# indygreg/python-zstandard

Hardware: AMD Instinct MI355X
Metric: GB/s uncompressed throughput, batch decompress of 128 KiB level-3 frames (the decompress half of BASELINE.json's metric; the compress half on the same inputs is this line's 'compress' object) (higher is better)
Workload: dtype u8

## Files before the change

python-zstandard_amd/csrc/zhip_decode_kernel.hpp:

```cpp
#pragma once
#include "zhip_device.hpp"
#include "zhip_format.hpp"
#include "zhip_xxh64.hpp"

#if defined(ZHIP_EMU) && defined(ZD_TRACE)
#include <stdio.h>
extern "C" { extern long zd_trace_pos; extern long zd_cur_frame; extern long zd_stat[16]; }
#define ZD_STAT(i, v) do { if (zh_lane() == 0) zd_stat[i] += (v); } while (0)
#define ZD_TRR(lo, n, what, a1, a2) do { if (zh_lane() == 0 && zd_trace_pos + 40 >= (long)(lo) && zd_trace_pos < (long)(lo) + (long)(n) + 40) fprintf(stderr, "[trace] f%ld range [%ld,+%ld) %s %ld %ld\n", zd_cur_frame, (long)(lo), (long)(n), what, (long)(a1), (long)(a2)); } while (0)
#define ZD_TR(pos, what, a1, a2, a3) do { if ((long)(pos) == zd_trace_pos) fprintf(stderr, "[trace] f%ld pos=%ld %s lane=%u %ld %ld %ld\n", zd_cur_frame, (long)(pos), what, zh_lane(), (long)(a1), (long)(a2), (long)(a3)); } while (0)
#else
#define ZD_TR(pos, what, a1, a2, a3) do { } while (0)
#define ZD_TRR(lo, n, what, a1, a2) do { } while (0)
#define ZD_STAT(i, v) do { } while (0)
#endif
#define ZD_STAGE_BYTES 512
#define ZD_ASM_BYTES 4096
#define ZD_COOP_LEN 32

ZH_CONST uint32_t zc_llBase[36] = {0,1,2,3,4,5,6,7,8,9,10,11,12,13,14,15,16,18,20,22,24,28,32,40,48,64,128,256,512,
                                   1024,2048,4096,8192,16384,32768,65536};
ZH_CONST uint8_t zc_llBits[36] = {0,0,0,0,0,0,0,0,0,0,0,0,0,0,0,0,1,1,1,1,2,2,3,3,4,6,7,8,9,10,11,12,13,14,15,16};
ZH_CONST uint32_t zc_mlBase[53] = {3,4,5,6,7,8,9,10,11,12,13,14,15,16,17,18,19,20,21,22,23,24,25,26,27,28,29,30,31,32,
                                   33,34,35,37,39,41,43,47,51,59,67,83,99,131,259,515,1027,2051,4099,8195,16387,32771,65539};
// ... 254 lines not shown
}
ZH_DEV bool zd_pb_init(ZdPBits& b, const uint8_t* src, uint32_t size)
{
    b.start = src; b.end = src + size; b.ptr = src; b.c = 0; b.d = 0; b.used = 64;
    if (size == 0) return false;
    const uint32_t last = src[size - 1];
    if (last == 0) return false;
    const uint32_t pad = 8 - (uint32_t)zh_highbit32(last);
    if (size >= 8) { b.ptr = src + size - 8; b.c = zh_ld64(b.ptr); b.used = pad; }
    else {
        uint64_t c = 0;
        for (uint32_t i = 0; i < size; i++) c |= (uint64_t)src[i] << (8 * i);
        b.c = c; b.used = pad + (8 - size) * 8;
    }
    b.d = zd_pb_below(b);
    return true;
}
ZH_DEV void zd_pb_norm(ZdPBits& b)
{
    uint32_t nb = b.used >> 3;
    const uint32_t room = (uint32_t)(b.ptr - b.start);
    if (nb > room) nb = room;
    if (nb > 8) nb = 8;
    if (nb) {
        b.c = nb == 8 ? b.d : ((b.c << (8 * nb)) | (b.d >> (64 - 8 * nb)));
        b.ptr -= nb; b.used -= nb * 8;
        b.d = zd_pb_below(b);
    }
}
ZH_DEV uint32_t zd_pb_peek(const ZdPBits& b, uint32_t n) { return (uint32_t)((b.c << (b.used & 63)) >> (64 - n)); }
ZH_DEV bool zd_pb_done(const ZdPBits& b) { return b.ptr == b.start && b.used == 64; }

ZH_DEV bool zd_weights_dist_ok(uint32_t tl, uint32_t maxS) { return tl <= 6 && maxS <= 12 && !(tl == 6 && maxS == 12); }
ZH_DEVFN int zd_read_huf_weights(ZdLDS& L, const uint8_t* src, uint32_t srcSize, uint32_t* pCount, uint32_t* pLog, const ZpPre* pre = nullptr, uint32_t at = 0)
{
    const uint32_t lane = zh_lane();
    if (srcSize < 1) return -ZE_CORRUPTION;
    uint32_t hb = src[0], n, used;
    if (hb >= 128) {
        n = hb - 127; used = 1 + (n + 1) / 2;
        if (used > srcSize) return -ZE_CORRUPTION;
        for (uint32_t i = lane; i < n; i += 64) {
            uint32_t v = src[1 + i / 2];
            L.weights[i] = (uint8_t)((i & 1) ? (v & 15) : (v >> 4));
        }
    } else {
        used = 1 + hb;
        if (used > srcSize || hb < 2) return -ZE_CORRUPTION;
        if (pre && pre->wCount && pre->wAt == at) {
            n = pre->wCount;
            zh_sync();
            ((uint32_t*)L.weights)[lane] = ((const uint32_t*)pre->weights)[lane];
#ifdef ZHIP_EMU
            if (lane == 0) zd_stat[10]++;
#endif
        } else {
        uint8_t* const stg = (uint8_t*)L.u.huf + 4096;
        zh_sync();
        zd_stage_wave(stg, src + 1, hb);
        zh_sync();
        if (lane == 0) {
            uint32_t maxS = 255 > 63 ? 63 : 255, tl = 0;
            int r = zd_read_ncount(L, stg, stg + hb, &maxS, &tl);
            L.misc[0] = (uint32_t)r; L.misc[1] = maxS; L.misc[2] = tl;
        }
        zh_sync();
// ... 3 lines not shown
        if (lane == 0) {
            ZdBits b; uint32_t cnt = 0; int bad = 0;
            if (!zd_bits_init(b, stg + r, hb - (uint32_t)r)) bad = 1;
            else {
                zd_bits_reload(b);
                uint32_t s1 = zd_bits_peek(b, tl); b.used += tl;
                uint32_t s2 = zd_bits_peek(b, tl); b.used += tl;
                if (tl == 0) { s1 = s2 = 0; }
                int64_t left;
                for (;;) {
                    if (b.used >= 32) zd_bits_reload(b);
                    left = (int64_t)(b.ptr - b.start) * 8 + 64 - (int64_t)b.used;
                    uint32_t e1 = L.u.b.wfse[s1], nb1 = (e1 >> 10) & 15;
                    if (cnt > 253) { bad = 1; break; }
                    L.weights[cnt++] = (uint8_t)(e1 >> 19);
                    uint32_t v1 = nb1 ? zd_bits_peek(b, nb1) : 0; b.used += nb1; left -= nb1;
                    s1 = (e1 & 1023) + v1;
                    uint32_t e2 = L.u.b.wfse[s2], nb2 = (e2 >> 10) & 15;
                    if (left < 0) { L.weights[cnt++] = (uint8_t)(e2 >> 19); break; }
                    if (cnt > 253) { bad = 1; break; }
                    L.weights[cnt++] = (uint8_t)(e2 >> 19);
                    uint32_t v2 = nb2 ? zd_bits_peek(b, nb2) : 0; b.used += nb2; left -= nb2;
                    s2 = (e2 & 1023) + v2;
                    if (left < 0) { L.weights[cnt++] = (uint8_t)(L.u.b.wfse[s1] >> 19); break; }
                }
            }
            L.misc[0] = bad ? 0xFFFFFFFFu : cnt;
        }
        zh_sync();
        n = L.misc[0];
        if (n == 0xFFFFFFFFu || n == 0) return -ZE_CORRUPTION;
        }
    }
    zh_sync();
    uint32_t part = 0, ones = 0;
    for (uint32_t i = lane; i < n; i += 64) {
        uint32_t w = L.weights[i];
        if (w > 12) part = 0x02000000u;
        else if (w) part += 1u << (w - 1);
        ones += (w == 1);
    }
    uint32_t total = zh_shfl(zh_scan_add(part), 63);
    uint32_t nOnes = zh_shfl(zh_scan_add(ones), 63);
    if (total == 0 || total >= 0x02000000u) return -ZE_CORRUPTION;
    uint32_t log = (uint32_t)zh_highbit32(total) + 1;
    if (log > 12) return -ZE_CORRUPTION;
    uint32_t rest = (1u << log) - total;
    if (rest & (rest - 1)) return -ZE_CORRUPTION;
    uint32_t lastW = (uint32_t)zh_highbit32(rest) + 1;
    nOnes += (lastW == 1);
    if (nOnes < 2 || (nOnes & 1)) return -ZE_CORRUPTION;
    if (lane == 0) L.weights[n] = (uint8_t)lastW;
    zh_sync();
    *pCount = n + 1; *pLog = log;
    return (int)used;
}

ZH_DEVFN int zd_build_huf(ZdLDS& L, uint32_t count)
{
    const uint32_t lane = zh_lane();
    const uint64_t lt = zh_lt_mask();
    uint32_t wt[4], myStart[4];
    uint32_t part = 0;
    for (int k = 0; k < 4; k++) {
        uint32_t s = (uint32_t)k * 64 + lane;
        wt[k] = s < count ? L.weights[s] : 0;
        if (wt[k]) part += 1u << (wt[k] - 1);
        myStart[k] = 0;
    }
    uint32_t total = zh_shfl(zh_scan_add(part), 63);
    if (total == 0 || (total & (total - 1))) return -ZE_CORRUPTION;
    uint32_t log = (uint32_t)zh_highbit32(total);
    if (log > 12 || log == 0) return -ZE_CORRUPTION;
    zh_sync();
    uint32_t base = 0;
    for (uint32_t w = 1; w <= 12; w++) {
        uint32_t before = 0;
        for (int k = 0; k < 4; k++) {
            uint64_t m = zh_ballot(wt[k] == w);
            if (wt[k] == w) myStart[k] = base + ((before + (uint32_t)zh_popc64(m & lt)) << (w - 1));
            before += (uint32_t)zh_popc64(m);
        }
        base += before << (w - 1);
    }
    for (int k = 0; k < 4; k++) {
        if (!wt[k]) continue;
        uint32_t len = 1u << (wt[k] - 1);
// ... 144 lines not shown
ZH_DEVFN int zd_seq_table(ZdLDS& L, uint32_t mode, int kind, uint32_t* pLog, const uint8_t* p, const uint8_t* end, const ZpPre* pre = nullptr)
{
    const uint32_t lane = zh_lane();
    uint32_t* table = L.fse + (kind == ZD_KIND_LL ? ZD_FSE_LL : kind == ZD_KIND_ML ? ZD_FSE_ML : ZD_FSE_OF);
    const uint32_t maxSym = kind == ZD_KIND_LL ? ZF_MAXLL : kind == ZD_KIND_ML ? ZF_MAXML : ZF_MAXOFF;
    const uint32_t maxLog = kind == ZD_KIND_LL ? ZF_LL_LOGMAX : kind == ZD_KIND_ML ? ZF_ML_LOGMAX : ZF_OF_LOGMAX;
    if (mode == 0) {
        zh_sync();
        if (kind == ZD_KIND_LL) L.norm[lane] = lane < 36 ? zc_llDef[lane] : (int16_t)0;
        else if (kind == ZD_KIND_ML) L.norm[lane] = lane < 53 ? zc_mlDef[lane] : (int16_t)0;
        else L.norm[lane] = lane < 29 ? zc_ofDef[lane] : (int16_t)0;
        uint32_t lg = kind == ZD_KIND_OF ? 5 : 6;
        uint32_t ms = kind == ZD_KIND_LL ? 35 : kind == ZD_KIND_ML ? 52 : 28;
        if (zd_build_fse(L, table, ms, lg, kind) < 0) return -ZE_CORRUPTION;
        *pLog = lg; return 0;
    }
    if (mode == 1) {
        if (p >= end) return -ZE_SRC_SIZE_WRONG;
        uint32_t s = p[0];
        if (s > maxSym) return -ZE_CORRUPTION;
        zh_sync();
        if (lane == 0) {
            uint32_t extra = kind == ZD_KIND_LL ? L.llBits[s] : kind == ZD_KIND_ML ? L.mlBits[s] : s;
            table[0] = ZD_CELL(0, 0, extra, s);
        }
        zh_sync();
        *pLog = 0; return 1;
    }
    if (mode == 2) {
        zh_sync();
        int r; uint32_t ms, tl;
        if (pre && pre->t[kind].valid) {
            L.norm[lane] = pre->norm[kind][lane];
            r = (int)pre->t[kind].used; ms = pre->t[kind].maxSym; tl = pre->t[kind].log;
#ifdef ZHIP_EMU
            if (lane == 0) zd_stat[11]++;
#endif
        } else {
            if (lane == 0) {
                uint32_t ms0 = maxSym, tl0 = 0;
                int r0 = zd_read_ncount(L, p, end, &ms0, &tl0);
                L.misc[0] = (uint32_t)r0; L.misc[1] = ms0; L.misc[2] = tl0;
            }
            zh_sync();
            r = (int)L.misc[0]; ms = L.misc[1]; tl = L.misc[2];
        }
        if (r < 0 || tl > maxLog) return -ZE_CORRUPTION;
        if (zd_build_fse(L, table, ms, tl, kind) < 0) return -ZE_CORRUPTION;
        *pLog = tl; return r;
    }
    if (*pLog == 0xFF) return -ZE_CORRUPTION;
    return 0;
}

ZH_DEV uint32_t zd_hist_byte(const uint8_t* dst, const uint8_t* dictEnd, int32_t pos)
{
    return pos >= 0 ? dst[pos] : dictEnd[pos];
}

ZH_COLD void zd_match_wave(uint8_t* dst, const uint8_t* dictEnd, uint32_t mdst, uint32_t off, uint32_t ml)
{
    const uint32_t lane = zh_lane();
    const int32_t sbeg = (int32_t)mdst - (int32_t)off;
    if (off >= 64) {
        for (uint32_t c = 0; c < ml; c += 64) {
            uint32_t j = c + lane;
            if (j < ml) dst[mdst + j] = (uint8_t)zd_hist_byte(dst, dictEnd, sbeg + (int32_t)j);
// ... 492 lines not shown
```

python-zstandard_amd/csrc/zhip_decode_pipeline.hpp:

```cpp
#pragma once
#include "zhip_decode_kernel.hpp"

ZH_DEV void zp_pack_fse(ZdLDS& L, uint32_t* T, uint32_t llLog, uint32_t ofLog, uint32_t mlLog)
{
    const uint32_t lane = zh_lane();
    for (uint32_t u = lane; u < ZP_FSE_CELLS / 2; u += 64) {
        const uint32_t lg = u < 256 ? llLog : u < 512 ? mlLog : ofLog;
        const uint32_t local = (2 * u) & (u < 512 ? 511u : 255u);
        uint32_t pair = 0;
        for (uint32_t k = 0; k < 2; k++) {
            uint32_t cell = 0;
            if (local + k < (1u << lg)) {
                const uint32_t e = L.fse[2 * u + k];
                cell = ((e >> 19) << 10) | (((e & 1023) + (1u << lg)) >> ((e >> 10) & 15));
            }
            pair |= cell << (16 * k);
        }
        T[u] = pair;
    }
}

struct ZpHdr { uint32_t pos, blockMax, hasChecksum, skippable; uint64_t fcs; };
ZH_DEV int zp_frame_header(const ZhipPipeArgs& a, const uint8_t* src, uint32_t srcSize, ZpHdr& h)
{
    const uint32_t mg = a.magicless ? 0u : 4u;
    h.skippable = 0;
    if (srcSize < mg + 1) return ZE_SRC_SIZE_WRONG;
    if (mg && (zh_ld32(src) & 0xFFFFFFF0u) == ZF_MAGIC_SKIPPABLE) {
        if (srcSize < 8 || (uint64_t)zh_ld32(src + 4) + 8 > srcSize) return ZE_SRC_SIZE_WRONG;
        h.skippable = 1; h.pos = 0; h.blockMax = 0; h.hasChecksum = 0; h.fcs = 0;
        return 0;
    }
    if (mg && zh_ld32(src) != ZF_MAGIC) return ZE_PREFIX_UNKNOWN;
    const uint32_t fhd = src[mg];
// ... 76 lines not shown
        if (modes & 3) return ZE_CORRUPTION;
        const bool allShared = share && de && (modes >> 2) == 0x3F;
        if (allShared) {
            st.llLog = de->llLog; st.ofLog = de->ofLog; st.mlLog = de->mlLog;
            if (sp >= send) return ZE_CORRUPTION;
        } else {
            if (de && !dictInLds) {
                zh_sync();
                const uint32_t* T = a.dictTables->fse;
                if ((modes >> 6) == 3) { for (uint32_t k = lane; k < (1u << de->llLog); k += 64) L.fse[ZD_FSE_LL + k] = T[ZD_FSE_LL + k]; st.llLog = de->llLog; }
                if (((modes >> 4) & 3) == 3) { for (uint32_t k = lane; k < (1u << de->ofLog); k += 64) L.fse[ZD_FSE_OF + k] = T[ZD_FSE_OF + k]; st.ofLog = de->ofLog; }
                if (((modes >> 2) & 3) == 3) { for (uint32_t k = lane; k < (1u << de->mlLog); k += 64) L.fse[ZD_FSE_ML + k] = T[ZD_FSE_ML + k]; st.mlLog = de->mlLog; }
                zh_sync();
            }
            const uint32_t hn = (uint32_t)(send - sp) < 256u ? (uint32_t)(send - sp) : 256u;
            uint8_t* const stg = (uint8_t*)L.u.huf + 4096;
            zh_sync();
            zd_stage_wave(stg, sp, hn);
            zh_sync();
            const uint8_t* lp = stg; const uint8_t* const lend = stg + hn;
            const ZpPre* const spre = df.pre && df.pre->seqAt == (uint32_t)(sp - (src + pos)) ? df.pre : nullptr;
            int q = zd_seq_table(L, modes >> 6, ZD_KIND_LL, &st.llLog, lp, lend, spre); if (q < 0) return -q; sp += q; lp += q;
            q = zd_seq_table(L, (modes >> 4) & 3, ZD_KIND_OF, &st.ofLog, lp, lend, spre); if (q < 0) return -q; sp += q; lp += q;
            q = zd_seq_table(L, (modes >> 2) & 3, ZD_KIND_ML, &st.mlLog, lp, lend, spre); if (q < 0) return -q; sp += q; lp += q;
            if (sp >= send) return ZE_CORRUPTION;
            zh_sync();
            uint32_t* const T = (uint32_t*)(a.fseTables + (size_t)t * ZP_FSE_CELLS);
            zp_pack_fse(L, T, st.llLog, st.ofLog, st.mlLog);
        }
        m.logs = st.llLog | (st.ofLog << 8) | (st.mlLog << 16) | (allShared ? ZP_LOGS_SHARED : 0u);
    }
    m.seqOff = (uint32_t)(sp - src); m.seqEnd = pos + bs;
    ZD_T(P, ZP_SEQTAB);
    return 0;
}

ZH_DEV void zp_enter_bins(const ZhipPipeArgs& a, ZdMeta& m)
{
    const uint32_t ks = m.nbSeq ? 1u + (m.nbSeq >> ZP_BIN_SHIFT) : 0u;
    const uint32_t kl = (m.litMode & 255u) == 3u ? 1u + (m.litSize >> ZP_LITBIN_SHIFT) : 0u;
    if (ks) m.pad = zh_atomic_add(a.counters + ZP_CNT_BINS + (256 - (ks > 256 ? 256u : ks)), 1u);
    if (kl) m.hasChecksum |= zh_atomic_add(a.counters + ZP_CNT_BINS + 256 + (256 - (kl > 256 ? 256u : kl)), 1u) << 1;
}
ZH_DEV void zp_enter_bins_wave(const ZhipPipeArgs& a, ZdMeta& m, bool on)
{
    const uint32_t lane = zh_lane();
    const uint32_t ks = on && m.nbSeq ? 1u + (m.nbSeq >> ZP_BIN_SHIFT) : 0u;
    const uint32_t kl = on && (m.litMode & 255u) == 3u ? 1u + (m.litSize >> ZP_LITBIN_SHIFT) : 0u;
    const uint32_t bS = ks ? 256u - (ks > 256u ? 256u : ks) : 0xFFFFu, bL = kl ? 256u + (256u - (kl > 256u ? 256u : kl)) : 0xFFFFu;
#pragma unroll
    for (int which = 0; which < 2; which++) {
        const uint32_t mine = which ? bL : bS;
        uint64_t todo = zh_ballot(mine != 0xFFFFu);
        while (todo) {
            const uint32_t leader = (uint32_t)zh_ctz64(todo);
            const uint32_t b = zh_shfl(mine, leader);
            const uint64_t same = zh_ballot(mine == b);
            uint32_t base = 0;
            if (lane == leader) base = zh_atomic_add(a.counters + ZP_CNT_BINS + b, (uint32_t)zh_popc64(same));
            base = zh_shfl(base, leader);
            if (mine == b) { const uint32_t rank = base + (uint32_t)zh_popc64(same & zh_lt_mask()); if (which) m.hasChecksum |= rank << 1; else m.pad = rank; }
            todo &= ~same;
        }
    }
}
ZH_DEV void zp_meta_clear(ZdMeta& m)
// ... 87 lines not shown
        const bool done = mine && zp_lit_shared_try(a, a.first + i, m, need16);
        const uint32_t n16 = done ? need16 : 0u;
        const uint32_t incl = zh_scan_add(n16), total = zh_shfl(incl, 63);
        uint32_t lb = 0;
        if (total) lb = zh_first(zh_atomic_add(a.counters + 8, lane == 0 ? total : 0u)) + incl - n16;
        const bool noRoom = done && n16 && (uint64_t)lb + n16 > a.arenaBudget16;
        zp_enter_bins_wave(a, m, done && !noRoom);
        if (a.ckLater) {
            const uint32_t nck = (uint32_t)zh_popc64(zh_ballot(done && !noRoom && (m.hasChecksum & 1u)));
            anyCk |= nck != 0;
        }
        if (done) {
            if (noRoom) {
                const uint32_t bm = m.blockMax, lo = m.fcsLo, hi = m.fcsHi;
                zp_meta_clear(m); m.blockMax = bm; m.fcsLo = lo; m.fcsHi = hi; m.path = 2;
                a.meta[i] = m;
                const uint32_t k = zh_atomic_add(a.fallbackCount, 1u); a.fallbackList[k] = a.first + i;
            } else {
                a.bases[2 * (size_t)i + 1] = n16 ? a.arenaBudget16 - lb - n16 : 0u;
                a.meta[i] = m;
#ifdef ZHIP_EMU
                zd_stat[7]++;
#endif
            }
        }
        const uint64_t rest = zh_ballot(mine && !done);
        if (rest) {
            const uint32_t at = zh_first(zh_atomic_add(a.counters + 10, lane == 0 ? (uint32_t)zh_popc64(rest) : 0u));
            if (mine && !done) a.order[at + (uint32_t)zh_popc64(rest & zh_lt_mask())] = i;
        }
    }
}

struct ZpPreLane { int16_t wnorm[64]; uint16_t cell[64]; uint8_t symAt[64]; uint8_t next[16]; uint32_t pad; };
struct ZpPreLDS { ZpPreLane lane[64]; };

ZH_DEV void zp_pre_weights(ZpPre& R, ZpPreLane& S, const uint8_t* desc, uint32_t hb, uint32_t at)
{
    uint32_t maxS = 63, tl = 0;
    const int r = zd_read_ncount_to(S.wnorm, desc, desc + hb, &maxS, &tl);
    if (r < 0 || !zd_weights_dist_ok(tl, maxS)) return;
    const uint32_t size = 1u << tl, mask = size - 1, step = (size >> 1) + (size >> 3) + 3;
    uint32_t high = size - 1, total = 0;
    for (uint32_t q = 0; q <= maxS; q++) {
        const int n = S.wnorm[q];
        if (n == -1) { S.symAt[high--] = (uint8_t)q; S.next[q] = 1; total++; }
        else { S.next[q] = (uint8_t)n; total += (uint32_t)n; }
    }
    if (total != size) return;
    uint32_t pos = 0;
    for (uint32_t q = 0; q <= maxS; q++) {
        const int n = S.wnorm[q];
        for (int k = 0; k < n; k++) {
            S.symAt[pos] = (uint8_t)q;
            do pos = (pos + step) & mask; while (pos > high);
        }
    }
    for (uint32_t u = 0; u < size; u++) {
        const uint32_t q = S.symAt[u], x = S.next[q];
        S.next[q] = (uint8_t)(x + 1);
        const uint32_t nb = tl - (uint32_t)zh_highbit32(x);
        S.cell[u] = (uint16_t)(((x << nb) - size) | (nb << 6) | (q << 9));
    }
    ZdBits b; uint32_t cnt = 0;
    if (!zd_bits_init(b, desc + r, hb - (uint32_t)r)) return;
    zd_bits_reload(b);
    uint32_t s1 = zd_bits_peek(b, tl); b.used += tl;
    uint32_t s2 = zd_bits_peek(b, tl); b.used += tl;
    if (tl == 0) { s1 = s2 = 0; }
    int64_t left;
    for (;;) {
        if (b.used >= 32) zd_bits_reload(b);
        left = (int64_t)(b.ptr - b.start) * 8 + 64 - (int64_t)b.used;
        const uint32_t e1 = S.cell[s1], nb1 = (e1 >> 6) & 7;
        if (cnt > 253) return;
        R.weights[cnt++] = (uint8_t)(e1 >> 9);
        const uint32_t v1 = nb1 ? zd_bits_peek(b, nb1) : 0; b.used += nb1; left -= nb1;
        s1 = (e1 & 63) + v1;
        const uint32_t e2 = S.cell[s2], nb2 = (e2 >> 6) & 7;
        if (left < 0) { R.weights[cnt++] = (uint8_t)(e2 >> 9); break; }
        if (cnt > 253) return;
        R.weights[cnt++] = (uint8_t)(e2 >> 9);
        const uint32_t v2 = nb2 ? zd_bits_peek(b, nb2) : 0; b.used += nb2; left -= nb2;
        s2 = (e2 & 63) + v2;
        if (left < 0) { R.weights[cnt++] = (uint8_t)(S.cell[s1] >> 9); break; }
    }
    R.wAt = at; R.wCount = cnt;
}

ZH_DEV void zp_pre_one(const ZhipPipeArgs& a, uint32_t f, ZpPre& R, ZpPreLane& S)
{
    R.wCount = 0; R.wAt = 0; R.seqAt = 0; R.t[0].valid = 0; R.t[1].valid = 0; R.t[2].valid = 0;
    const uint8_t* src = a.src + a.srcSegs[2 * (size_t)f];
    const uint64_t srcSize64 = a.srcSegs[2 * (size_t)f + 1];
    if (srcSize64 > 0x7FFFFFFFull) return;
    const uint32_t srcSize = (uint32_t)srcSize64;
    ZpHdr h;
    if (zp_frame_header(a, src, srcSize, h) || h.skippable) return;
    uint32_t pos = h.pos;
    if (pos + 3 > srcSize) return;
    const uint32_t bh = zh_ld24(src + pos); pos += 3;
    const uint32_t bs = bh >> 3;
    if (!(bh & 1) || ((bh >> 1) & 3) != 2) return;
    if (pos + bs > srcSize || bs > h.blockMax || bs < 2) return;
    const uint8_t* const b = src + pos;
    const uint32_t b0 = b[0], lt = b0 & 3, fmt = (b0 >> 2) & 3;
    uint32_t used, regen;
    if (lt < 2) {
        uint32_t hdr;
        if (fmt == 1) { hdr = 2; regen = zh_ld16(b) >> 4; }
        else if (fmt == 3) { if (bs < 3) return; hdr = 3; regen = zh_ld24(b) >> 4; }
        else { hdr = 1; regen = b0 >> 3; }
        if (regen > h.blockMax) return;
        if (lt == 0) { if (hdr + regen > bs) return; used = hdr + regen; }
        else { if (hdr + 1 > bs) return; used = hdr + 1; }
    } else {
        if (bs < 5) return;
        const uint32_t v = zh_ld32(b);
        uint32_t hdr, four, csize;
        if (fmt < 2) { hdr = 3; four = fmt; regen = (v >> 4) & 0x3FF; csize = (v >> 14) & 0x3FF; }
        else if (fmt == 2) { hdr = 4; four = 1; regen = (v >> 4) & 0x3FFF; csize = v >> 18; }
        else { hdr = 5; four = 1; regen = (v >> 4) & 0x3FFFF; csize = (v >> 22) + ((uint32_t)b[4] << 10); }
        if (regen > h.blockMax || regen > ZF_BLOCK_MAX) return;
        if (four ? regen < 6 : regen == 0) return;
        if (hdr + csize > bs) return;
        used = hdr + csize;
        if (lt == 2 && csize >= 1) {
            const uint32_t hb = b[hdr];
            if (hb >= 2 && hb < 128 && 1 + hb <= csize) zp_pre_weights(R, S, b + hdr + 1, hb, hdr);
        }
    }
    uint32_t sp = used; const uint32_t send = bs;
    if (sp >= send) return;
    uint32_t nbSeq = b[sp++];
    if (nbSeq > 127) {
        if (nbSeq == 255) { if (sp + 2 > send) return; nbSeq = zh_ld16(b + sp) + 0x7F00; sp += 2; }
        else { if (sp >= send) return; nbSeq = ((nbSeq - 128) << 8) + b[sp++]; }
    }
    if (nbSeq == 0 || nbSeq > ZP_SEQ_CAP - 16 || sp >= send) return;
    const uint32_t modes = b[sp++];
    if (modes & 3) return;
    const uint32_t hn = send - sp < 256u ? send - sp : 256u;
    const uint8_t* lp = b + sp; const uint8_t* const lend = lp + hn;
    R.seqAt = sp;
#pragma unroll
    for (int kind = 0; kind < 3; kind++) {
        const uint32_t mode = kind == ZD_KIND_LL ? modes >> 6 : kind == ZD_KIND_OF ? (modes >> 4) & 3 : (modes >> 2) & 3;
        if (mode == 3) return;
        if (mode == 1) { if (lp >= lend) return; lp += 1; }
        if (mode == 2) {
            uint32_t ms = kind == ZD_KIND_LL ? ZF_MAXLL : kind == ZD_KIND_ML ? ZF_MAXML : ZF_MAXOFF, tl = 0;
            const int r = zd_read_ncount_to(R.norm[kind], lp, lend, &ms, &tl);
            if (r < 0) return;
            R.t[kind].maxSym = ms; R.t[kind].log = tl; R.t[kind].used = (uint32_t)r; R.t[kind].valid = 1;
            lp += r;
        }
    }
}

ZH_DEVFN void zp_pre_body(const ZhipPipeArgs& a, ZpPreLDS& L)
{
    const uint32_t lane = zh_lane();
    for (;;) {
        const uint32_t base = zh_first(zh_atomic_add(a.counters + 11, lane == 0 ? 64u : 0u));
        if (base >= a.count) break;
        const uint32_t i = base + lane;
        if (i < a.count) zp_pre_one(a, a.first + i, a.pre[i], L.lane[lane]);
    }
}

ZH_DEVFN void zp_lit_body(const ZhipPipeArgs& a, ZdLDS& L)
{
    const uint32_t lane = zh_lane();
    if (lane < 36) { L.llBase[lane] = zc_llBase[lane]; L.llBits[lane] = zc_llBits[lane]; }
    if (lane < 53) { L.mlBase[lane] = zc_mlBase[lane]; L.mlBits[lane] = zc_mlBits[lane]; }
    zh_sync();
    bool anyCk = false;
    for (;;) {
        const uint32_t got = zh_atomic_add(a.counters + 0, lane == 0 ? 1u : 0u);
        if (zh_opaque(lane) == 0) L.misc[7] = got;
        zh_sync();
        const uint32_t got1 = zh_first(L.misc[7]);
        zh_sync();
        if (got1 >= (a.k1Lanes ? a.counters[10] : a.count)) { if (anyCk && zh_opaque(lane) == 0) *(volatile uint32_t*)(a.counters + 12) = 1u; break; }
        const uint32_t i = a.k1Lanes ? a.order[got1] : got1;
        const uint32_t f = a.first + i;
        ZdMeta m;
        zp_meta_clear(m);
        const uint8_t* src = a.src + a.srcSegs[2 * (size_t)f];
        const uint64_t srcSize64 = a.srcSegs[2 * (size_t)f + 1];
        uint8_t* dst = a.dst + a.dstSegs[2 * (size_t)f];
        const uint64_t cap64 = a.dstSegs[2 * (size_t)f + 1];
        int err = 0; bool fallback = false;
        ZdProf P; P.on = a.prof != nullptr;
        if (P.on) { for (int q = 0; q < ZP_N; q++) P.acc[q] = 0; P.t0 = zd_clock(); }
        do {
            if (srcSize64 > 0x7FFFFFFFull) { fallback = true; break; }
            const uint32_t srcSize = (uint32_t)srcSize64;
            const uint32_t cap = cap64 > 0x7FFFFFFFull ? 0x7FFFFFFFu : (uint32_t)cap64;
            ZpHdr h;
            err = zp_frame_header(a, src, srcSize, h);
            if (err || h.skippable) break;
            const uint32_t blockMax = h.blockMax, hasChecksum = h.hasChecksum;
            const uint64_t fcs = h.fcs;
            uint32_t pos = h.pos;
            m.blockMax = blockMax; m.fcsLo = (uint32_t)fcs; m.fcsHi = (uint32_t)(fcs >> 32);
            if (pos + 3 > srcSize) { err = ZE_SRC_SIZE_WRONG; break; }
            const uint32_t bh = zh_ld24(src + pos); pos += 3;
            const uint32_t lastBlock = bh & 1, type = (bh >> 1) & 3, bs = bh >> 3;
            if (!lastBlock) { fallback = true; break; }
            if (type == 3) { err = ZE_CORRUPTION; break; }
            const bool onePass = fcs != ~0ull && cap64 >= fcs;
            if (type < 2) {
                if (type == 0 ? pos + bs > srcSize : pos + 1 > srcSize) { err = ZE_SRC_SIZE_WRONG; break; }
                if (bs > blockMax && !onePass) { err = ZE_CORRUPTION; break; }
                if (bs > cap) { err = ZE_DST_TOO_SMALL; break; }
                if (type == 0) zd_copy_wave(dst, src + pos, bs); else zd_fill_wave(dst, src[pos], bs);
                if (fcs != ~0ull && fcs != bs) { err = ZE_CORRUPTION; break; }
                m.produced = bs;
                if (hasChecksum && a.ckLater) {
                    const uint32_t cpos = pos + (type == 0 ? bs : 1);
                    if (cpos + 4 > srcSize) { err = ZE_CHECKSUM_WRONG; break; }
                    m.hasChecksum = 1; m.checksum = zh_ld32(src + cpos);
                    anyCk = true;
                } else if (hasChecksum) {
                    const uint32_t cpos = pos + (type == 0 ? bs : 1);
                    if (cpos + 4 > srcSize) { err = ZE_CHECKSUM_WRONG; break; }
                    zd_fence();
                    zh_sync();
// ... 8 lines not shown
            if (pos + bs > srcSize) { err = ZE_SRC_SIZE_WRONG; break; }
            if (bs > blockMax) { err = onePass ? ZE_SRC_SIZE_WRONG : ZE_CORRUPTION; break; }
            if (bs < 2) { err = ZE_CORRUPTION; break; }
            ZdState st;
            st.rep0 = 1; st.rep1 = 4; st.rep2 = 8; st.hufCount = 0; st.llLog = st.ofLog = st.mlLog = 0xFF;
            ZD_T(P, ZP_HEADER);
            ZdLitDefer df; df.table = a.hufTables + (size_t)i * ZP_HUF_CELLS; df.maxLog = ZP_HUF_LOGMAX; df.taken = 0;
            df.log = 0; df.four = 0; df.streamBytes = 0; df.streams = src; df.prevTable = nullptr; df.prevLog = 0; df.shared = 0; df.shareOK = 1;
            df.pre = a.pre ? a.pre + i : nullptr;
            const ZhipDictEntropy* const de = a.dictEntropy;
            if (de) {
                st.hufCount = de->hufCount;
                if (a.dictTables->hufLog <= ZP_HUF_LOGMAX) { df.prevTable = a.dictTables->huf; df.prevLog = a.dictTables->hufLog; }
                else {
                    zh_sync(); for (uint32_t k = lane; k < 256; k += 64) L.weights[k] = de->hufWeights[k]; zh_sync();
#ifdef ZHIP_EMU
                    if (lane == 0) zd_stat[6]++;
#endif
                }
            }
            err = zp_block_tables(a, L, st, df, src, pos, bs, blockMax, i, m, P, true, false);
            if (err == (int)ZP_RC_FALLBACK) { err = 0; fallback = true; break; }
            if (err) break;
            if (hasChecksum) {
                if (pos + bs + 4 > srcSize) { err = ZE_CHECKSUM_WRONG; break; }
                m.hasChecksum = 1; m.checksum = zh_ld32(src + pos + bs);
                anyCk = anyCk || a.ckLater != 0;
            }
            m.path = 1;
        } while (false);
        if (fallback) { m.path = 2; }
        if (err) { m.status = err; m.path = 0; }
        zh_sync();
        if (zh_opaque(lane) == 0) {
            if (m.path == 1) zp_enter_bins(a, m);
            a.meta[i] = m;
            if (m.path == 2) { const uint32_t k = zh_atomic_add(a.fallbackCount, 1u); a.fallbackList[k] = f; }
            if (m.path == 0) { a.status[f] = m.status; a.outSizes[f] = m.status ? 0 : m.produced; }
        }
#ifdef ZHIP_EMU
        zd_fence();
#endif
        if (P.on) { ZD_T(P, ZP_RAW); if (lane == 0) for (int q = 0; q < ZP_N; q++) if (P.acc[q]) zh_atomic_add64(a.prof + q, P.acc[q]); }
    }
}

ZH_DEVFN void zp_lit_mb_body(const ZhipPipeArgs& a, ZdLDS& L)
{
    const uint32_t lane = zh_lane();
    if (lane < 36) { L.llBase[lane] = zc_llBase[lane]; L.llBits[lane] = zc_llBits[lane]; }
    if (lane < 53) { L.mlBase[lane] = zc_mlBase[lane]; L.mlBits[lane] = zc_mlBits[lane]; }
    zh_sync();
    bool anyCk = false;
    for (;;) {
        const uint32_t got = zh_atomic_add(a.counters + 0, lane == 0 ? 1u : 0u);
        if (zh_opaque(lane) == 0) L.misc[7] = got;
        zh_sync();
        const uint32_t i = zh_first(L.misc[7]);
        zh_sync();
        if (i >= a.count) { if (anyCk && zh_opaque(lane) == 0) *(volatile uint32_t*)(a.counters + 12) = 1u; break; }
        const uint32_t f = a.first + i;
        const uint8_t* src = a.src + a.srcSegs[2 * (size_t)f];
        const uint64_t srcSize64 = a.srcSegs[2 * (size_t)f + 1];
        const uint64_t cap64 = a.dstSegs[2 * (size_t)f + 1];
        ZpFrameRec rec; rec.firstItem = 0; rec.nItems = 0; rec.path = 0; rec.blockMax = 0; rec.fcsLo = rec.fcsHi = 0xFFFFFFFFu; rec.hasChecksum = 0; rec.checksum = 0;
        int err = 0; bool fallback = false;
// ... 1080 lines not shown
```

python-zstandard_amd/csrc/zhip_format.hpp:

```cpp
#pragma once
#include <stdint.h>

enum {
    ZE_OK = 0, ZE_GENERIC = 1, ZE_PREFIX_UNKNOWN = 10, ZE_FRAMEPARAM_UNSUPPORTED = 14, ZE_WINDOW_TOO_LARGE = 16,
    ZE_CORRUPTION = 20, ZE_CHECKSUM_WRONG = 22, ZE_LITERALS_HEADER_WRONG = 24, ZE_DICT_CORRUPTED = 30,
    ZE_DICT_WRONG = 32, ZE_PARAM_UNSUPPORTED = 40, ZE_PARAM_OUTOFBOUND = 42, ZE_TABLELOG_TOO_LARGE = 44, ZE_MAXSYMBOL_TOO_LARGE = 46,
    ZE_MAXSYMBOL_TOO_SMALL = 48, ZE_MEMORY = 64, ZE_DST_TOO_SMALL = 70, ZE_SRC_SIZE_WRONG = 72, ZE_SEQ_INVALID = 107
};

#define ZF_MAGIC 0xFD2FB528u
#define ZF_MAGIC_SKIPPABLE 0x184D2A50u
#define ZF_DICT_MAGIC 0xEC30A437u
#define ZF_BLOCK_MAX (1u << 17)
#define ZF_MAXLL 35
#define ZF_MAXML 52
#define ZF_MAXOFF 31
#define ZF_LL_LOGMAX 9
#define ZF_ML_LOGMAX 9
#define ZF_OF_LOGMAX 8

#define ZHIP_LIT_STRIDE (ZF_BLOCK_MAX + 256)

struct ZhipDictEntropy {
    uint8_t  hufWeights[256];
    uint32_t hufCount;
    int16_t  ofNorm[32]; uint32_t ofMax, ofLog;
    int16_t  mlNorm[53]; uint32_t mlMax, mlLog;
    int16_t  llNorm[36]; uint32_t llMax, llLog;
    uint32_t rep[3];
    uint32_t contentOffset;
    uint32_t dictID;
    int32_t  status;
};

// ... 153 lines not shown
#define ZP_SEQ_OFBITS 29
#define ZP_LIT_STRIDE ((size_t)ZF_BLOCK_MAX + 256)
#define ZP_LIT_FRONT 256u
#define ZP_FSE_LL 0
#define ZP_FSE_ML 512
#define ZP_FSE_OF 1024
#define ZP_FSE_CELLS 1280
#define ZP_K2_STRIDE 2564
#define ZP_HUF_LOGMAX 11
#define ZP_HUF_CELLS (1u << ZP_HUF_LOGMAX)
#ifndef ZP_HUF_FRAMES
#define ZP_HUF_FRAMES 12
#endif
#define ZP_HUF_LS (ZP_HUF_FRAMES > 8 ? 6 : ZP_HUF_FRAMES > 4 ? 5 : 4)
#define ZP_LITBIN_SHIFT 9
#define ZP_BIN_SHIFT 7

#define ZP_CNT_BINS 16u
#define ZP_CNT_WORDS (16u + 512u)

struct ZpFrameRec {
    uint32_t firstItem, nItems;
    uint32_t path;
    uint32_t blockMax;
    uint32_t fcsLo, fcsHi;
    uint32_t hasChecksum, checksum;
};
#define ZP_OF_LIMIT 0x1E000000u
#define ZP_SYM_REP(k) (0x1E800000u + ((uint32_t)(k) << 23))
#define ZP_SYM_TOP ZP_SYM_REP(2)
#define ZP_MB_MAXBLOCKS 4096u
#define ZP_RC_FALLBACK 0x7FFF0002
struct alignas(16) ZpPre {
    uint8_t weights[256];
    int16_t norm[3][64];
    uint32_t wCount;
    uint32_t wAt;
    struct { uint32_t valid, maxSym, log, used; } t[3];
    uint32_t seqAt;
    uint32_t pad;
};
struct ZhipPipeArgs {
    const uint8_t* src; const uint64_t* srcSegs;
    uint8_t* dst; const uint64_t* dstSegs;
    uint64_t* outSizes; int32_t* status;
    ZdMeta* meta;
    uint8_t* litArena;
    uint64_t* seqArena;
    uint32_t* bases;
    uint32_t arenaBudget16;
    uint16_t* fseTables;
    uint32_t* order;
    uint16_t* hufTables;
    uint32_t* orderLit;
    uint32_t* counters;
    uint32_t* fallbackCount;
    uint32_t* fallbackList;
    uint32_t first, count;
    uint32_t itemCap;
    uint32_t* itemFrame;
    uint32_t* itemReps;
    ZpFrameRec* frameRecs;
    uint64_t maxWindowSize;
    uint32_t magicless;
    uint32_t ckLater;
    ZpPre* pre;
    uint32_t k1Lanes;
    unsigned long long* prof;
    uint32_t dictID, dictContentSize;
    const uint8_t* dictContent;
    const ZhipDictEntropy* dictEntropy;
    const ZhipDictTables* dictTables;
};
```

Measured before the change: 407.0.

## Let the header kernel decode blocks from a precomputed per-frame record

The pre-pass kernel now stores a complete 64-byte block header record (literal type, sizes, modes, checksum, frame fields) next to the Huffman weights and FSE distributions whenever the block is a single-block frame it can fully describe. The first pipeline kernel reads that record with wave-uniform loads and builds the Huffman and FSE tables straight from it, so it no longer re-parses the frame and block headers from global memory. The ZpPre layout is repacked with 16/8-bit fields into a fixed 704-byte shape. Optional LDS staging in the pre-pass and a fetch-ahead work counter are added but stay off by default. This adds a second decode path that must stay consistent with the full parser, and non-qualifying blocks fall back to the old path.

Result: no change. 409.8, median of 6 (+0.7%).

```diff
diff --git a/python-zstandard_amd/csrc/zhip_decode_kernel.hpp b/python-zstandard_amd/csrc/zhip_decode_kernel.hpp
--- a/python-zstandard_amd/csrc/zhip_decode_kernel.hpp
+++ b/python-zstandard_amd/csrc/zhip_decode_kernel.hpp
@@ -310,6 +310,32 @@
 ZH_DEV bool zd_pb_done(const ZdPBits& b) { return b.ptr == b.start && b.used == 64; }
 
 ZH_DEV bool zd_weights_dist_ok(uint32_t tl, uint32_t maxS) { return tl <= 6 && maxS <= 12 && !(tl == 6 && maxS == 12); }
+ZH_DEV int zd_huf_last_weight(ZdLDS& L, uint32_t n, uint32_t* pCount, uint32_t* pLog)
+{
+    const uint32_t lane = zh_lane();
+    zh_sync();
+    uint32_t part = 0, ones = 0;
+    for (uint32_t i = lane; i < n; i += 64) {
+        uint32_t w = L.weights[i];
+        if (w > 12) part = 0x02000000u;
+        else if (w) part += 1u << (w - 1);
+        ones += (w == 1);
+    }
+    uint32_t total = zh_shfl(zh_scan_add(part), 63);
+    uint32_t nOnes = zh_shfl(zh_scan_add(ones), 63);
+    if (total == 0 || total >= 0x02000000u) return -ZE_CORRUPTION;
+    uint32_t log = (uint32_t)zh_highbit32(total) + 1;
+    if (log > 12) return -ZE_CORRUPTION;
+    uint32_t rest = (1u << log) - total;
+    if (rest & (rest - 1)) return -ZE_CORRUPTION;
+    uint32_t lastW = (uint32_t)zh_highbit32(rest) + 1;
+    nOnes += (lastW == 1);
+    if (nOnes < 2 || (nOnes & 1)) return -ZE_CORRUPTION;
+    if (lane == 0) L.weights[n] = (uint8_t)lastW;
+    zh_sync();
+    *pCount = n + 1; *pLog = log;
+    return 0;
+}
 ZH_DEVFN int zd_read_huf_weights(ZdLDS& L, const uint8_t* src, uint32_t srcSize, uint32_t* pCount, uint32_t* pLog, const ZpPre* pre = nullptr, uint32_t at = 0)
 {
     const uint32_t lane = zh_lane();
@@ -379,27 +405,7 @@
         if (n == 0xFFFFFFFFu || n == 0) return -ZE_CORRUPTION;
         }
     }
-    zh_sync();
-    uint32_t part = 0, ones = 0;
-    for (uint32_t i = lane; i < n; i += 64) {
-        uint32_t w = L.weights[i];
-        if (w > 12) part = 0x02000000u;
-        else if (w) part += 1u << (w - 1);
-        ones += (w == 1);
-    }
-    uint32_t total = zh_shfl(zh_scan_add(part), 63);
-    uint32_t nOnes = zh_shfl(zh_scan_add(ones), 63);
-    if (total == 0 || total >= 0x02000000u) return -ZE_CORRUPTION;
-    uint32_t log = (uint32_t)zh_highbit32(total) + 1;
-    if (log > 12) return -ZE_CORRUPTION;
-    uint32_t rest = (1u << log) - total;
-    if (rest & (rest - 1)) return -ZE_CORRUPTION;
-    uint32_t lastW = (uint32_t)zh_highbit32(rest) + 1;
-    nOnes += (lastW == 1);
-    if (nOnes < 2 || (nOnes & 1)) return -ZE_CORRUPTION;
-    if (lane == 0) L.weights[n] = (uint8_t)lastW;
-    zh_sync();
-    *pCount = n + 1; *pLog = log;
+    if (zd_huf_last_weight(L, n, pCount, pLog) < 0) return -ZE_CORRUPTION;
     return (int)used;
 }
 
@@ -610,7 +616,7 @@
         int r; uint32_t ms, tl;
         if (pre && pre->t[kind].valid) {
             L.norm[lane] = pre->norm[kind][lane];
-            r = (int)pre->t[kind].used; ms = pre->t[kind].maxSym; tl = pre->t[kind].log;
+            r = (int)pre->used[kind]; ms = pre->t[kind].maxSym; tl = pre->t[kind].log;
 #ifdef ZHIP_EMU
             if (lane == 0) zd_stat[11]++;
 #endif
diff --git a/python-zstandard_amd/csrc/zhip_decode_pipeline.hpp b/python-zstandard_amd/csrc/zhip_decode_pipeline.hpp
--- a/python-zstandard_amd/csrc/zhip_decode_pipeline.hpp
+++ b/python-zstandard_amd/csrc/zhip_decode_pipeline.hpp
@@ -1,5 +1,15 @@
 #pragma once
 #include "zhip_decode_kernel.hpp"
+
+#ifndef ZP_K1_RECORD
+#define ZP_K1_RECORD 1
+#endif
+#ifndef ZP_K0_LDS
+#define ZP_K0_LDS 0
+#endif
+#ifndef ZP_K1_AHEAD
+#define ZP_K1_AHEAD 0
+#endif
 
 ZH_DEV void zp_pack_fse(ZdLDS& L, uint32_t* T, uint32_t llLog, uint32_t ofLog, uint32_t mlLog)
 {
@@ -142,6 +152,78 @@
     }
     m.seqOff = (uint32_t)(sp - src); m.seqEnd = pos + bs;
     ZD_T(P, ZP_SEQTAB);
+    return 0;
+}
+
+ZH_DEV int zp_block_from_record(const ZhipPipeArgs& a, ZdLDS& L, const ZpPre* pre, const uint32_t* hd, uint32_t t, ZdMeta& m, ZdProf& P)
+{
+    const uint32_t lane = zh_lane();
+    const uint32_t flags = hd[7], lt = (flags >> 1) & 3u, four = (flags >> 3) & 1u, modes = (flags >> 8) & 255u, pos = (flags >> 16) & 255u;
+    const uint32_t wCount = hd[0] & 0xFFFFu, seqAt = hd[1], nbSeq = hd[6] >> 16, bs = hd[8], regen = hd[12], csize = hd[13], hdr = hd[15] & 255u, hb = hd[15] >> 8;
+    const uint32_t need16 = lt == 2 ? (regen + 256u + 15u) >> 4 : 0u;
+    uint32_t lb = 0;
+    if (need16) lb = zh_atomic_add(a.counters + 8, lane == 0 ? need16 : 0u);
+    uint32_t w4 = 0;
+    if (lt == 2) w4 = ((const uint32_t*)pre->weights)[lane];
+    int16_t nv[3] = { 0, 0, 0 };
+#pragma unroll
+    for (int kind = 0; kind < 3; kind++) if (((modes >> (kind == ZD_KIND_LL ? 6 : kind == ZD_KIND_OF ? 4 : 2)) & 3u) == 2u) nv[kind] = pre->norm[kind][lane];
+    if (lt == 2) {
+        zh_sync();
+        ((uint32_t*)L.weights)[lane] = w4;
+        uint32_t cnt = 0, wl = 0;
+        int e = zd_huf_last_weight(L, wCount, &cnt, &wl) < 0 ? (int)ZE_CORRUPTION : 0;
+        int lg = 0;
+        if (!e) { lg = zd_build_huf(L, cnt); if (lg < 0) e = ZE_CORRUPTION; }
+        lb = zh_first(lb);
+        if ((uint64_t)lb + need16 > a.arenaBudget16) {
+            if (zh_opaque(lane) == 0) zh_atomic_add(a.counters + 8, 0u - need16);
+            return ZP_RC_FALLBACK;
+        }
+        if (e) return e;
+        if ((uint32_t)lg > ZP_HUF_LOGMAX) return ZP_RC_FALLBACK;
+        const uint32_t left = csize - 1u - hb;
+        if (four && (left < 10 || 3 * ((regen + 3) / 4) > regen)) return ZE_CORRUPTION;
+        const uint64_t* t8 = (const uint64_t*)L.u.huf; uint64_t* g8 = (uint64_t*)(a.hufTables + (size_t)t * ZP_HUF_CELLS);
+        for (uint32_t i = lane; i < (1u << lg) / 4 + ((1u << lg) < 4 ? 1u : 0u); i += 64) g8[i] = t8[i];
+        m.litMode = 3u | ((uint32_t)lg << 8) | (four << 16); m.litOff = pos + hdr + 1u + hb; m.produced = left;
+#ifdef ZHIP_EMU
+        if (lane == 0) zd_stat[10]++;
+#endif
+    } else if (lt == 1) { m.litMode = 2; m.litOff = flags >> 24; }
+    else { m.litMode = 0; m.litOff = pos + hdr; }
+    m.litSize = regen;
+    if (zh_opaque(lane) == 0) a.bases[2 * (size_t)t + 1] = need16 ? a.arenaBudget16 - lb - need16 : 0u;
+    ZD_T(P, ZP_HUFTAB);
+    m.nbSeq = nbSeq;
+    uint32_t logs[3] = { 0xFF, 0xFF, 0xFF }, sp = seqAt;
+#pragma unroll
+    for (int k3 = 0; k3 < 3; k3++) {
+        const int kind = k3 == 0 ? ZD_KIND_LL : k3 == 1 ? ZD_KIND_OF : ZD_KIND_ML;
+        const uint32_t mode = (modes >> (6 - 2 * k3)) & 3u;
+        if (mode == 2) {
+            const uint32_t tl = (hd[2 + kind] >> 16) & 255u, ms = (hd[2 + kind] >> 8) & 255u;
+            const uint32_t maxLog = kind == ZD_KIND_LL ? ZF_LL_LOGMAX : kind == ZD_KIND_ML ? ZF_ML_LOGMAX : ZF_OF_LOGMAX;
+            zh_sync();
+            L.norm[lane] = nv[kind];
+            if (tl > maxLog) return ZE_CORRUPTION;
+            if (zd_build_fse(L, L.fse + (kind == ZD_KIND_LL ? ZD_FSE_LL : kind == ZD_KIND_ML ? ZD_FSE_ML : ZD_FSE_OF), ms, tl, kind) < 0) return ZE_CORRUPTION;
+            logs[kind] = tl;
+            sp += (hd[5 + (kind >> 1)] >> (16 * (kind & 1))) & 0xFFFFu;
+#ifdef ZHIP_EMU
+            if (lane == 0) zd_stat[11]++;
+#endif
+        } else if (zd_seq_table(L, 0, kind, &logs[kind], nullptr, nullptr) < 0) return ZE_CORRUPTION;
+    }
+    if (sp >= bs) return ZE_CORRUPTION;
+    zh_sync();
+    zp_pack_fse(L, (uint32_t*)(a.fseTables + (size_t)t * ZP_FSE_CELLS), logs[ZD_KIND_LL], logs[ZD_KIND_OF], logs[ZD_KIND_ML]);
+    m.logs = logs[ZD_KIND_LL] | (logs[ZD_KIND_OF] << 8) | (logs[ZD_KIND_ML] << 16);
+    m.seqOff = pos + sp; m.seqEnd = pos + bs;
+    ZD_T(P, ZP_SEQTAB);
+#ifdef ZHIP_EMU
+    if (lane == 0) zd_stat[3]++;
+#endif
     return 0;
 }
 
@@ -295,10 +377,24 @@
     }
 }
 
+#if ZP_K0_LDS
+struct ZpPreLane { int16_t wnorm[64]; uint16_t cell[64]; uint8_t symAt[64]; uint8_t next[16]; uint32_t strip[64]; uint32_t pad; };
+#else
 struct ZpPreLane { int16_t wnorm[64]; uint16_t cell[64]; uint8_t symAt[64]; uint8_t next[16]; uint32_t pad; };
+#endif
 struct ZpPreLDS { ZpPreLane lane[64]; };
-
-ZH_DEV void zp_pre_weights(ZpPre& R, ZpPreLane& S, const uint8_t* desc, uint32_t hb, uint32_t at)
+#if ZP_K0_LDS
+ZH_DEV void zp_pre_stage(uint32_t* strip, uint32_t at, const uint8_t* p, const uint8_t* end, uint32_t n)
+{
+    uint64_t v[16];
+#pragma unroll
+    for (uint32_t k = 0; k < 16; k++) v[k] = 8 * k < n ? zd_ld64_bounded(p + 8 * k, end) : 0ull;
+#pragma unroll
+    for (uint32_t k = 0; k < 16; k++) if (8 * k < n) { strip[at / 4 + 2 * k] = (uint32_t)v[k]; strip[at / 4 + 2 * k + 1] = (uint32_t)(v[k] >> 32); }
+}
+#endif
+
+ZH_DEV void zp_pre_weights(ZpPre& R, ZpPreLane& S, const uint8_t* desc, uint32_t hb, uint32_t at, uint32_t* pSum)
 {
     uint32_t maxS = 63, tl = 0;
     const int r = zd_read_ncount_to(S.wnorm, desc, desc + hb, &maxS, &tl);
@@ -325,7 +421,7 @@
         const uint32_t nb = tl - (uint32_t)zh_highbit32(x);
         S.cell[u] = (uint16_t)(((x << nb) - size) | (nb << 6) | (q << 9));
     }
-    ZdBits b; uint32_t cnt = 0;
+    ZdBits b; uint32_t cnt = 0, sum = 0;
     if (!zd_bits_init(b, desc + r, hb - (uint32_t)r)) return;
     zd_bits_reload(b);
     uint32_t s1 = zd_bits_peek(b, tl); b.used += tl;
@@ -337,23 +433,23 @@
         left = (int64_t)(b.ptr - b.start) * 8 + 64 - (int64_t)b.used;
         const uint32_t e1 = S.cell[s1], nb1 = (e1 >> 6) & 7;
         if (cnt > 253) return;
-        R.weights[cnt++] = (uint8_t)(e1 >> 9);
+        R.weights[cnt++] = (uint8_t)(e1 >> 9); sum += (1u << (e1 >> 9)) >> 1;
         const uint32_t v1 = nb1 ? zd_bits_peek(b, nb1) : 0; b.used += nb1; left -= nb1;
         s1 = (e1 & 63) + v1;
         const uint32_t e2 = S.cell[s2], nb2 = (e2 >> 6) & 7;
-        if (left < 0) { R.weights[cnt++] = (uint8_t)(e2 >> 9); break; }
+        if (left < 0) { R.weights[cnt++] = (uint8_t)(e2 >> 9); sum += (1u << (e2 >> 9)) >> 1; break; }
         if (cnt > 253) return;
-        R.weights[cnt++] = (uint8_t)(e2 >> 9);
+        R.weights[cnt++] = (uint8_t)(e2 >> 9); sum += (1u << (e2 >> 9)) >> 1;
         const uint32_t v2 = nb2 ? zd_bits_peek(b, nb2) : 0; b.used += nb2; left -= nb2;
         s2 = (e2 & 63) + v2;
-        if (left < 0) { R.weights[cnt++] = (uint8_t)(S.cell[s1] >> 9); break; }
-    }
-    R.wAt = at; R.wCount = cnt;
+        if (left < 0) { const uint32_t w = S.cell[s1] >> 9; R.weights[cnt++] = (uint8_t)w; sum += (1u << w) >> 1; break; }
+    }
+    R.wAt = (uint16_t)at; R.wCount = (uint16_t)cnt; *pSum = sum;
 }
 
 ZH_DEV void zp_pre_one(const ZhipPipeArgs& a, uint32_t f, ZpPre& R, ZpPreLane& S)
 {
-    R.wCount = 0; R.wAt = 0; R.seqAt = 0; R.t[0].valid = 0; R.t[1].valid = 0; R.t[2].valid = 0;
+    R.wCount = 0; R.wAt = 0; R.seqAt = 0; R.t[0].valid = 0; R.t[1].valid = 0; R.t[2].valid = 0; R.flags = 0;
     const uint8_t* src = a.src + a.srcSegs[2 * (size_t)f];
     const uint64_t srcSize64 = a.srcSegs[2 * (size_t)f + 1];
     if (srcSize64 > 0x7FFFFFFFull) return;
@@ -368,19 +464,18 @@
     if (pos + bs > srcSize || bs > h.blockMax || bs < 2) return;
     const uint8_t* const b = src + pos;
     const uint32_t b0 = b[0], lt = b0 & 3, fmt = (b0 >> 2) & 3;
-    uint32_t used, regen;
+    uint32_t used, regen, hdr, four = 0, csize = 0, hb = 0, rleByte = 0;
+    bool whole = true;
     if (lt < 2) {
-        uint32_t hdr;
         if (fmt == 1) { hdr = 2; regen = zh_ld16(b) >> 4; }
         else if (fmt == 3) { if (bs < 3) return; hdr = 3; regen = zh_ld24(b) >> 4; }
         else { hdr = 1; regen = b0 >> 3; }
         if (regen > h.blockMax) return;
         if (lt == 0) { if (hdr + regen > bs) return; used = hdr + regen; }
-        else { if (hdr + 1 > bs) return; used = hdr + 1; }
+        else { if (hdr + 1 > bs) return; used = hdr + 1; rleByte = b[hdr]; }
     } else {
         if (bs < 5) return;
         const uint32_t v = zh_ld32(b);
-        uint32_t hdr, four, csize;
         if (fmt < 2) { hdr = 3; four = fmt; regen = (v >> 4) & 0x3FF; csize = (v >> 14) & 0x3FF; }
         else if (fmt == 2) { hdr = 4; four = 1; regen = (v >> 4) & 0x3FFF; csize = v >> 18; }
         else { hdr = 5; four = 1; regen = (v >> 4) & 0x3FFFF; csize = (v >> 22) + ((uint32_t)b[4] << 10); }
@@ -389,9 +484,15 @@
         if (hdr + csize > bs) return;
         used = hdr + csize;
         if (lt == 2 && csize >= 1) {
-            const uint32_t hb = b[hdr];
-            if (hb >= 2 && hb < 128 && 1 + hb <= csize) zp_pre_weights(R, S, b + hdr + 1, hb, hdr);
-        }
+            hb = b[hdr];
+            uint32_t sum = 0;
+#if ZP_K0_LDS
+            if (hb >= 2 && hb < 128 && 1 + hb <= csize) { zp_pre_stage(S.strip, 0, b + hdr + 1, b + hdr + 1 + hb, hb); zp_pre_weights(R, S, (const uint8_t*)S.strip, hb, hdr, &sum); }
+#else
+            if (hb >= 2 && hb < 128 && 1 + hb <= csize) zp_pre_weights(R, S, b + hdr + 1, hb, hdr, &sum);
+#endif
+            if (!R.wCount || sum == 0 || (uint32_t)zh_highbit32(sum) + 1 > ZP_HUF_LOGMAX) whole = false;
+        } else whole = false;
     }
     uint32_t sp = used; const uint32_t send = bs;
     if (sp >= send) return;
@@ -404,21 +505,36 @@
     const uint32_t modes = b[sp++];
     if (modes & 3) return;
     const uint32_t hn = send - sp < 256u ? send - sp : 256u;
+#if ZP_K0_LDS
+    zp_pre_stage(S.strip, 0, b + sp, b + sp + hn, hn < 128u ? hn : 128u);
+    if (hn > 128u) zp_pre_stage(S.strip, 128, b + sp + 128, b + sp + hn, hn - 128u);
+    const uint8_t* lp = (const uint8_t*)S.strip; const uint8_t* const lend = lp + hn;
+#else
     const uint8_t* lp = b + sp; const uint8_t* const lend = lp + hn;
+#endif
     R.seqAt = sp;
 #pragma unroll
     for (int kind = 0; kind < 3; kind++) {
         const uint32_t mode = kind == ZD_KIND_LL ? modes >> 6 : kind == ZD_KIND_OF ? (modes >> 4) & 3 : (modes >> 2) & 3;
         if (mode == 3) return;
-        if (mode == 1) { if (lp >= lend) return; lp += 1; }
+        if (mode == 1) { if (lp >= lend) return; lp += 1; whole = false; }
+        R.used[kind] = 0;
         if (mode == 2) {
             uint32_t ms = kind == ZD_KIND_LL ? ZF_MAXLL : kind == ZD_KIND_ML ? ZF_MAXML : ZF_MAXOFF, tl = 0;
             const int r = zd_read_ncount_to(R.norm[kind], lp, lend, &ms, &tl);
             if (r < 0) return;
-            R.t[kind].maxSym = ms; R.t[kind].log = tl; R.t[kind].used = (uint32_t)r; R.t[kind].valid = 1;
+            R.t[kind].maxSym = (uint8_t)ms; R.t[kind].log = (uint8_t)tl; R.used[kind] = (uint16_t)r; R.t[kind].valid = 1;
             lp += r;
         }
     }
+#if ZP_K1_RECORD
+    if (!whole) return;
+    uint32_t ck = 0;
+    if (h.hasChecksum) { if (pos + bs + 4 > srcSize) return; ck = zh_ld32(src + pos + bs); }
+    R.nbSeq = (uint16_t)nbSeq; R.blockSize = bs; R.blockMax = h.blockMax; R.fcsLo = (uint32_t)h.fcs; R.fcsHi = (uint32_t)(h.fcs >> 32);
+    R.regen = regen; R.csize = csize; R.checksum = ck; R.litHdr = hdr | (hb << 8);
+    R.flags = ZP_PRE_COMPLETE | (lt << 1) | (four << 3) | (h.hasChecksum << 4) | (modes << 8) | (pos << 16) | (rleByte << 24);
+#endif
 }
 
 ZH_DEVFN void zp_pre_body(const ZhipPipeArgs& a, ZpPreLDS& L)
@@ -439,12 +555,19 @@
     if (lane < 53) { L.mlBase[lane] = zc_mlBase[lane]; L.mlBits[lane] = zc_mlBits[lane]; }
     zh_sync();
     bool anyCk = false;
+#if ZP_K1_AHEAD
+    uint32_t ahead = zh_atomic_add(a.counters + 0, lane == 0 ? 1u : 0u);
+#endif
     for (;;) {
+#if ZP_K1_AHEAD
+        const uint32_t got1 = zh_first(ahead);
+#else
         const uint32_t got = zh_atomic_add(a.counters + 0, lane == 0 ? 1u : 0u);
         if (zh_opaque(lane) == 0) L.misc[7] = got;
         zh_sync();
         const uint32_t got1 = zh_first(L.misc[7]);
         zh_sync();
+#endif
         if (got1 >= (a.k1Lanes ? a.counters[10] : a.count)) { if (anyCk && zh_opaque(lane) == 0) *(volatile uint32_t*)(a.counters + 12) = 1u; break; }
         const uint32_t i = a.k1Lanes ? a.order[got1] : got1;
         const uint32_t f = a.first + i;
@@ -457,7 +580,28 @@
         int err = 0; bool fallback = false;
         ZdProf P; P.on = a.prof != nullptr;
         if (P.on) { for (int q = 0; q < ZP_N; q++) P.acc[q] = 0; P.t0 = zd_clock(); }
+#if ZP_K1_RECORD
+        uint32_t hd[16]; bool byRecord = false;
+        if (a.pre) {
+            const uint32_t* const hp = (const uint32_t*)(a.pre + i);
+#pragma unroll
+            for (int q = 0; q < 16; q++) hd[q] = zh_first(hp[q]);
+            byRecord = (hd[7] & ZP_PRE_COMPLETE) != 0;
+        }
+#endif
         do {
+#if ZP_K1_RECORD
+            if (byRecord) {
+                m.blockMax = hd[9]; m.fcsLo = hd[10]; m.fcsHi = hd[11];
+                ZD_T(P, ZP_HEADER);
+                err = zp_block_from_record(a, L, a.pre + i, hd, i, m, P);
+                if (err == (int)ZP_RC_FALLBACK) { err = 0; fallback = true; break; }
+                if (err) break;
+                if (hd[7] & 16u) { m.hasChecksum = 1; m.checksum = hd[14]; anyCk = anyCk || a.ckLater != 0; }
+                m.path = 1;
+                break;
+            }
+#endif
             if (srcSize64 > 0x7FFFFFFFull) { fallback = true; break; }
             const uint32_t srcSize = (uint32_t)srcSize64;
             const uint32_t cap = cap64 > 0x7FFFFFFFull ? 0x7FFFFFFFu : (uint32_t)cap64;
@@ -532,6 +676,9 @@
         if (fallback) { m.path = 2; }
         if (err) { m.status = err; m.path = 0; }
         zh_sync();
+#if ZP_K1_AHEAD
+        ahead = zh_atomic_add(a.counters + 0, lane == 0 ? 1u : 0u);
+#endif
         if (zh_opaque(lane) == 0) {
             if (m.path == 1) zp_enter_bins(a, m);
             a.meta[i] = m;
diff --git a/python-zstandard_amd/csrc/zhip_format.hpp b/python-zstandard_amd/csrc/zhip_format.hpp
--- a/python-zstandard_amd/csrc/zhip_format.hpp
+++ b/python-zstandard_amd/csrc/zhip_format.hpp
@@ -1,5 +1,6 @@
 #pragma once
 #include <stdint.h>
+#include <stddef.h>
 
 enum {
     ZE_OK = 0, ZE_GENERIC = 1, ZE_PREFIX_UNKNOWN = 10, ZE_FRAMEPARAM_UNSUPPORTED = 14, ZE_WINDOW_TOO_LARGE = 16,
@@ -219,14 +220,24 @@
 #define ZP_MB_MAXBLOCKS 4096u
 #define ZP_RC_FALLBACK 0x7FFF0002
 struct alignas(16) ZpPre {
+    uint16_t wCount;
+    uint16_t wAt;
+    uint32_t seqAt;
+    struct { uint8_t valid, maxSym, log, pad; } t[3];
+    uint16_t used[3];
+    uint16_t nbSeq;
+    uint32_t flags;
+    uint32_t blockSize;
+    uint32_t blockMax;
+    uint32_t fcsLo, fcsHi;
+    uint32_t regen, csize;
+    uint32_t checksum;
+    uint32_t litHdr;
     uint8_t weights[256];
     int16_t norm[3][64];
-    uint32_t wCount;
-    uint32_t wAt;
-    struct { uint32_t valid, maxSym, log, used; } t[3];
-    uint32_t seqAt;
-    uint32_t pad;
-};
+};
+#define ZP_PRE_COMPLETE 1u
+static_assert(sizeof(ZpPre) == 704 && offsetof(ZpPre, weights) == 64, "ZpPre: a 64-byte head, then the weights and the three distributions");
 struct ZhipPipeArgs {
     const uint8_t* src; const uint64_t* srcSegs;
     uint8_t* dst; const uint64_t* dstSegs;
```
